# OminiX-ai/OminiX-MLX

Hardware: AMD Instinct MI355X
Metric: decode_tokens_per_sec (higher is better)
Workload: dtype bf16

## Files before the change

include/omx.h:

```cpp
#ifndef OMX_H
#define OMX_H

#include <stddef.h>
#include <stdint.h>

#ifdef __cplusplus
extern "C" {
#endif

typedef enum omx_dtype_ {
    OMX_BOOL = 0, OMX_UINT8 = 1, OMX_UINT16 = 2, OMX_UINT32 = 3, OMX_UINT64 = 4,
    OMX_INT8 = 5, OMX_INT16 = 6, OMX_INT32 = 7, OMX_INT64 = 8,
    OMX_FLOAT16 = 9, OMX_FLOAT32 = 10, OMX_FLOAT64 = 11, OMX_BFLOAT16 = 12, OMX_COMPLEX64 = 13
} omx_dtype;

typedef void* omx_stream;

const char* omx_version(void);
int omx_experiments_built(void);
typedef void (*omx_error_handler_func)(const char* msg, void* data);
void omx_set_error_handler(omx_error_handler_func handler, void* data, void (*dtor)(void*));
const char* omx_last_error(void);
void omx_clear_error(void);
int omx_device_count(int* count);
// ... 200 lines not shown
int omx_debug_attn_step(omx_attn_step_dbg* a, omx_stream stream);
typedef struct omx_gemv_rows_seg_ { const void* w; const void* bias; void* out; int cols, ld; } omx_gemv_rows_seg;
typedef struct omx_gemv_rows_dbg_ {
    const void* x; int M, K, segmented;
    const void* w; const void* bias; const void* resid; const void* gate; int relu, N; void* out;
    omx_gemv_rows_seg seg[3]; int n_plain;
    const void* w_gate; const void* w_up; void* out_act; int half, ld_act, act_mode;
    const void* pre_norm_w; float pre_norm_eps;
    int route_rpw;
} omx_gemv_rows_dbg;
int omx_debug_gemv_rows(omx_gemv_rows_dbg* a, omx_stream stream);
int omx_qwen3_stream(omx_qwen3 m, omx_stream* s);
int omx_qwen3_step_bytes(omx_qwen3 m, int ctx, double* bytes);
int omx_qwen3_decode_path(omx_qwen3 m, int* path);
int omx_qwen3_debug_trace_step(omx_qwen3 m, unsigned long long* host, size_t n_words, int* blocks);
int omx_qwen3_time_step_kernels(omx_qwen3 m, int steps, float* us);
int omx_qwen3_debug_trace_engine(omx_qwen3 m, unsigned long long* host, size_t n_words, int* cus);
int omx_qwen3_debug_step_forms(omx_qwen3 m, int* forms);
int omx_qwen3_debug_raise_give_up(omx_qwen3 m);

int omx_quantize(void* packed, void* scales, void* biases, const void* w, int64_t rows, int cols, int group_size, int bits,
                 omx_dtype dtype, omx_stream stream);
int omx_dequantize(void* out, const void* packed, const void* scales, const void* biases , int64_t rows,
                   int cols, int group_size, int bits, omx_dtype dtype, omx_stream stream);
int omx_quantized_matmul(void* out, const void* x, const void* packed, const void* scales, const void* biases, int M, int N,
                         int K, int group_size, int bits, omx_dtype dtype, omx_stream stream);
int omx_quantized_linear_mfma(void* out, const void* x, const void* packed, const void* scales, const void* biases, const void* resid,
                              const void* gate, int M, int N, int K, int group_size, int bits, omx_stream stream);
int omx_quantized_linear_swiglu(void* out_plain, void* out_act, const void* x, const void* packed, const void* scales, const void* biases,
                                int M, int n_plain, int half, int K, int group_size, int bits, omx_stream stream);
// ... 196 lines not shown
```

ominix-mlx_amd/csrc/attn.hpp:

```cpp
#pragma once
#include "common.hpp"

namespace omx {

struct AttnDecodeArgs {
    const bf16_t* q;
    const bf16_t* k;
    const bf16_t* v;
    int64_t kv_batch_stride, kv_head_stride;
    int B, H, Hkv, Tk;
    float scale;
    int mask_mode;
    const void* mask;
    int nsplit;
    float* ws_o;
    float* ws_ml;
    bf16_t* out;
    int64_t q_bs, q_hs;
    int causal_tail;
};

constexpr int kAttnTraceWords = 16;
struct AttnStepArgs {
    const bf16_t* qkv;
    bf16_t* k;
    bf16_t* v;
    int64_t kv_head_stride;
    int H, Hkv, cap;
    float scale, eps;
    const bf16_t* q_norm_w;
    const bf16_t* k_norm_w;
    const float* rope_cur;
    const int* pos_ptr;
    const unsigned* seq_ptr;
    unsigned tag_mul, tag_add;
    int chunk;
    int nsplit;
// ... 6 lines not shown
    bf16_t* o_out;
    float* o_out_f32;
    int o_rows;
    int o_rpw, o_nhi;
    uint64_t* xg;
    const uint32_t* o_wq;
    const uint32_t* o_sb;
    int o_group;
    int f16;
    const bf16_t* gu_gate;
    const bf16_t* gu_up;
    const bf16_t* gu_norm_w;
    bf16_t* gu_out;
    int gu_rows;
    uint64_t* hg;
    const bf16_t* dn_w;
    bf16_t* dn_out;
    uint64_t* ag;
    uint64_t* rg;
    const bf16_t* nq_w0;
    const bf16_t* nq_w1;
    const bf16_t* nq_w2;
    int nq_n0, nq_n1, nq_rows;
    const bf16_t* nq_norm_w;
    const bf16_t* nq_bias;
    bf16_t* nq_out;
};
bool attn_step_down_ok(int o_rows, int gu_rows, int nq_rows);
bool attn_step_oproj_ok(int H, int Hkv, int D, int nsplit, int o_rows);
bool attn_step_gateup_ok(int H, int Hkv, int D, int nsplit, int o_rows, int gu_rows);
// ... 12 lines not shown
```

ominix-mlx_amd/csrc/attn_step.hip:

```cpp
#include <algorithm>

#include "attn.hpp"
#include "act16.hpp"
#include "gemv_parts.hpp"
#include "granule.hpp"
#include "launch_timing.hpp"

namespace omx {

namespace {

constexpr int kBlock = 512;
constexpr int kWaves = 8;
constexpr unsigned kSpinLimit = 1u << 15;

template <int N>
__device__ __forceinline__ float swap_halves(float v) {
    if (N == 16) return dpp_f<0x128>(v);
    return dpp_f<0x1B>(dpp_f<kDppHalfMirror>(v));
}

template <bool F16 = false>
__device__ __forceinline__ void unpack8(const u32x4 r, float (&x)[8]) {
#pragma unroll
// ... 89 lines not shown
    return d;
}

__device__ __forceinline__ float dot8_chain(const u32x4 w, const u32x4 xp, float acc) {
#pragma unroll
    for (int i = 0; i < 4; ++i) {
        acc = fmaf(bf16lo(w[i]), bf16lo(xp[i]), acc);
        acc = fmaf(bf16hi(w[i]), bf16hi(xp[i]), acc);
    }
    return acc;
}

constexpr int kORows = 4;

constexpr int kGuBlockPairs = 48, kGuHidden = 4096, kGuNV = kGuHidden / 512;
enum { kGuTicket = 0, kGuReduced = 1, kGuWords = 4 };

__device__ __forceinline__ int gateup_claim(int* sm_gu, int lane) {
    int t = 0;
    if (lane == 0) t = __hip_atomic_fetch_add(sm_gu + kGuTicket, 1, __ATOMIC_RELAXED, __HIP_MEMORY_SCOPE_WORKGROUP);
    return __builtin_amdgcn_readfirstlane(t);
}

__device__ __forceinline__ void gateup_issue(const AttnStepArgs& a, u32x4 (*w)[kGuNV], int pair, int lane) {
    const u32x4* g = reinterpret_cast<const u32x4*>(a.gu_gate + (size_t)pair * kGuHidden);
    const u32x4* u = reinterpret_cast<const u32x4*>(a.gu_up + (size_t)pair * kGuHidden);
#pragma unroll
    for (int j = 0; j < kGuNV; ++j) {
        w[0][j] = ld_nt(g + j * 64 + lane);
        w[1][j] = ld_nt(u + j * 64 + lane);
    }
    __builtin_amdgcn_sched_barrier(0);
}

template <int NVW>
__device__ __forceinline__ void oproj_await_vector(const AttnStepArgs& a, u32x4* sm_x, unsigned tag, int lane, int wave) {
    asm volatile("s_waitcnt vmcnt(0)" ::: "memory");
    if (wave == 0) {
        constexpr int SEGS = NVW * 8;
        const uint64_t* probe = a.xg + (size_t)min(lane, SEGS - 1) * 32 + 31;
        for (unsigned spins = 0; spins < kSpinLimit; ++spins) {
            const unsigned long long g = ld_granule(probe);
            if (__all((unsigned)(g >> 32) == tag)) break;
            __builtin_amdgcn_s_sleep(4);
        }
    }
    __syncthreads();
// ... 255 lines not shown
            }
        if (TRACE) __hip_atomic_fetch_add(sm_gu + kDnStored, stored, __ATOMIC_RELAXED, __HIP_MEMORY_SCOPE_WORKGROUP);
    }
    if constexpr (TRACE) {
        lds_barrier();
        if (threadIdx.x == 0) {
            tr[14] = wall_clock64();
            tr[15] = (unsigned long long)sm_gu[kDnReduced] | (unsigned long long)sm_gu[kDnStored] << 32;
        }
    }
}

template <bool TRACE, bool DN = false>
__device__ __forceinline__ void gateup_phase(const AttnStepArgs& a, u32x4* xs, float* red, int* sm_gu, const uint16_t* sm_pub, unsigned tag,
                                             int lane, int wave, int pub_row0, int pub_rows, unsigned long long* tr,
                                             unsigned char* sm_dn = nullptr) {
    typedef Act16<false> A;
    const int pair0 = ((int)blockIdx.y * (int)gridDim.x + (int)blockIdx.x) * kGuBlockPairs;
    uint16_t* park = DN ? reinterpret_cast<uint16_t*>(sm_dn + kDnParkOff) : nullptr;
    constexpr int PV = kGuNV * 64 / 256;
    u32x4 nwv[PV];
#pragma unroll
    for (int i = 0; i < PV; ++i) nwv[i] = *(reinterpret_cast<const u32x4*>(a.gu_norm_w) + (threadIdx.x & 255) + i * 256);
    u32x4 wA[2][kGuNV], wB[2][kGuNV];
    int tA = 0, tB;
    if (wave != 0) {
        tA = gateup_claim(sm_gu, lane);
        gateup_issue(a, wA, pair0 + tA, lane);
    }
    lds_barrier();
    if (wave == 0) {
// ... 41 lines not shown
        gateup_issue(a, wB, pair0 + tB, lane);
    }
    lds_barrier();
    unsigned res2 = 0;
    if constexpr (DN) res2 = reinterpret_cast<const unsigned*>(xs)[(pair0 / kGuBlockPairs) * (kDnBlockRows / 2) + (lane & (kDnBlockRows / 2 - 1))];
    rmsnorm_in_lds<A, PV>(xs, red, nwv, kGuHidden, a.eps, threadIdx.x < 256);
    if (wave == 0) {
        gateup_issue(a, wB, pair0 + tB, lane);
        gateup_reduce<DN>(a, wA, xs, pair0 + tA, lane, park + tA);
        if (TRACE && threadIdx.x == 0) tr[7] = wall_clock64();
        asm volatile("; first pair reduced: wave 0, its second pair just asked for" ::: "memory");
    } else {
        gateup_reduce<DN>(a, wA, xs, pair0 + tA, lane, park + tA);
        asm volatile("; first pair reduced: the second pair came in through the hop" ::: "memory");
    }
    int n_reduced = 1;
    int nA = gateup_claim(sm_gu, lane), nB;
    for (;;) {
        if (nA >= kGuBlockPairs) {
            gateup_reduce<DN>(a, wB, xs, pair0 + tB, lane, park + tB);
            ++n_reduced;
            break;
        }
        tA = nA;
        gateup_issue(a, wA, pair0 + tA, lane);
        nB = gateup_claim(sm_gu, lane);
        gateup_reduce<DN>(a, wB, xs, pair0 + tB, lane, park + tB);
        if (nB >= kGuBlockPairs) {
            gateup_reduce<DN>(a, wA, xs, pair0 + tA, lane, park + tA);
            n_reduced += 2;
            break;
        }
        tB = nB;
        gateup_issue(a, wB, pair0 + tB, lane);
        nA = gateup_claim(sm_gu, lane);
        gateup_reduce<DN>(a, wA, xs, pair0 + tA, lane, park + tA);
        n_reduced += 2;
    }
    if constexpr (TRACE) {
        if (lane == 0) {
            __hip_atomic_fetch_add(sm_gu + kGuReduced, n_reduced, __ATOMIC_RELAXED, __HIP_MEMORY_SCOPE_WORKGROUP);
            if (wave == 0) tr[8] = wall_clock64();
            if (wave == kWaves - 1) tr[9] = wall_clock64();
        }
        lds_barrier();
        if (threadIdx.x == 0) tr[10] = (unsigned long long)sm_gu[kGuReduced];
    }
    if constexpr (DN) down_qkv_phase<TRACE>(a, sm_dn, xs, red, sm_gu, res2, tag, lane, wave, tr);
}

template <int NVW, int R, bool GU = false>
__device__ __forceinline__ void oproj_phase(const AttnStepArgs& a, u32x4* sm_x, unsigned tag, int lane, int wave, int o_row0,
                                            unsigned long long* tr, uint16_t* sm_pub = nullptr, int pub_row0 = 0) {
    u32x4 ow[R][NVW];
#pragma unroll
    for (int r = 0; r < R; ++r) {
        const int row = min(o_row0 + r, a.o_rows - 1);
        const u32x4* p = reinterpret_cast<const u32x4*>(a.o_w + (size_t)row * (NVW * 512));
#pragma unroll
        for (int j = 0; j < NVW; ++j) ow[r][j] = __builtin_nontemporal_load(p + j * 64 + lane);
    }
    bf16_t o_res[R];
#pragma unroll
    for (int r = 0; r < R; ++r) o_res[r] = a.o_resid[min(o_row0 + r, a.o_rows - 1)];
    __builtin_amdgcn_sched_barrier(0);
    oproj_await_vector<NVW>(a, sm_x, tag, lane, wave);
    if (tr && threadIdx.x == 0) tr[5] = wall_clock64();
    float acc[R];
#pragma unroll
    for (int r = 0; r < R; ++r) acc[r] = 0.f;
#pragma unroll
    for (int j = 0; j < NVW; ++j) {
        const u32x4 xp = sm_x[j * 64 + lane];
#pragma unroll
        for (int r = 0; r < R; ++r) acc[r] = dot8_chain(ow[r][j], xp, acc[r]);
    }
#pragma unroll
    for (int r = 0; r < R; ++r) acc[r] = wave_sum(acc[r]);
    if (lane == 0) {
#pragma unroll
// ... 105 lines not shown
    static_assert(!GU || (NVW == kGuNV && D == 128), "gate/up follows the bf16 O projection of hidden 4096 only");
    typedef Act16<F16> A16;
    constexpr int LPR = D / 8;
    constexpr int TPW = 64 / LPR;
    constexpr bool QO = NVW >= 100;
    constexpr int NV = QO ? NVW - 100 : NVW;
    constexpr bool OPROJ = NV > 0;
    extern __shared__ __attribute__((aligned(16))) unsigned char smem[];
    float* sm_o = reinterpret_cast<float*>(smem);
    float* sm_m = sm_o + kWaves * TPW * GT * D;
    float* sm_l = sm_m + kWaves * GT;
    u32x4* sm_q = reinterpret_cast<u32x4*>(sm_l + kWaves * GT);
    u32x4* sm_x = sm_q + (GT + 1) * LPR;
    float* sm_xsum = reinterpret_cast<float*>(sm_x + NV * 64);
    int* sm_gu = reinterpret_cast<int*>(sm_x + NV * 64);

    const int lane = threadIdx.x & 63;
    const int wave = threadIdx.x >> 6;
    const int c = lane % LPR;
    const int sg = lane / LPR;
    const int kvh = blockIdx.x, split = blockIdx.y;
    const int G = a.H / a.Hkv;
    unsigned long long* tr = TRACE ? a.trace + ((size_t)split * a.Hkv + kvh) * kAttnTraceWords : nullptr;
    if (TRACE && threadIdx.x == 0) tr[0] = wall_clock64();
    if constexpr (GU) {
        if (threadIdx.x < (DN ? kDnWords : kGuWords)) sm_gu[threadIdx.x] = 0;
    }

    bf16_t* Kb = a.k + (size_t)kvh * a.kv_head_stride;
    bf16_t* Vb = a.v + (size_t)kvh * a.kv_head_stride;
// ... 122 lines not shown
#pragma unroll
            for (int e = 0; e < 4; ++e) o[g][e] *= al;
#pragma unroll
            for (int u = 0; u < kKU; ++u) {
                const float p = (mn == -INFINITY) ? 0.f : __expf(s[u][g] - mn);
                l[g] += p;
                const f32x2 pp = {p, p};
#pragma unroll
                for (int e = 0; e < 4; ++e) o[g][e] = __builtin_elementwise_fma(pp, vf[u][e], o[g][e]);
            }
        }
    };
    if (wave < n_units && t_begin + wave * TPW < t_end) round(wave);
    for (int u0 = wave + kWaves * kKU; u0 < n_units && t_begin + u0 * TPW < t_end; u0 += kWaves * kKU) round(u0);
    if (TRACE && threadIdx.x == 0) tr[2] = wall_clock64();

    if (active) {
#pragma unroll
        for (int g = 0; g < GT; ++g) {
            float* dst = sm_o + (((size_t)(wave * TPW + sg) * GT + g) * D + c * 8);
            *reinterpret_cast<f32x4*>(dst) = f32x4{o[g][0][0], o[g][0][1], o[g][1][0], o[g][1][1]};
            *reinterpret_cast<f32x4*>(dst + 4) = f32x4{o[g][2][0], o[g][2][1], o[g][3][0], o[g][3][1]};
            float lw = readlane_f(l[g], 0);
#pragma unroll
            for (int r = 1; r < TPW; ++r) lw += readlane_f(l[g], r * LPR);
            if (lane == 0) {
                sm_m[wave * GT + g] = m[g];
                sm_l[wave * GT + g] = lw;
            }
        }
        __syncthreads();
        if (TRACE && !GU && threadIdx.x == 0) tr[7] = wall_clock64();
        for (int idx = threadIdx.x; idx < G * D; idx += kBlock) {
            const int g = idx / D, d = idx % D;
            float M = sm_m[g];
#pragma unroll
            for (int w = 1; w < kWaves; ++w) M = fmaxf(M, sm_m[w * GT + g]);
            float L = 0.f, O = 0.f;
#pragma unroll
            for (int w = 0; w < kWaves; ++w) {
                const float mw = sm_m[w * GT + g];
                const float f = (mw == -INFINITY) ? 0.f : __expf(mw - M);
                float ow = 0.f;
#pragma unroll
                for (int r = 0; r < TPW; ++r) ow += sm_o[((size_t)(w * TPW + r) * GT + g) * D + d];
                L = fmaf(f, sm_l[w * GT + g], L);
// ... 9 lines not shown
    }
    if (TRACE && threadIdx.x == 0) tr[3] = wall_clock64();

    if (OPROJ && split >= G) {
        const int g = ((split - G) * (int)gridDim.x + kvh) * kWaves + wave;
        const bool hi = g < a.o_nhi;
        const int rows = hi ? a.o_rpw : a.o_rpw - 1;
        const int o_row0 = hi ? g * a.o_rpw : a.o_nhi * a.o_rpw + (g - a.o_nhi) * (a.o_rpw - 1);
        unsigned long long* otr = TRACE ? tr : nullptr;
        if constexpr (GU) {
            auto row0_of = [&](int w) { return w < a.o_nhi ? w * a.o_rpw : a.o_nhi * a.o_rpw + (w - a.o_nhi) * (a.o_rpw - 1); };
            const int pub_row0 = row0_of(g - wave), pub_rows = row0_of(g - wave + kWaves) - pub_row0;
            uint16_t* sm_pub = reinterpret_cast<uint16_t*>(sm_l);
            if (rows == 2) oproj_phase<NV, 2, true>(a, sm_x, tag, lane, wave, o_row0, otr, sm_pub, pub_row0);
            else oproj_phase<NV, 3, true>(a, sm_x, tag, lane, wave, o_row0, otr, sm_pub, pub_row0);
            gateup_phase<TRACE, DN>(a, sm_x, sm_m, sm_gu, sm_pub, tag, lane, wave, pub_row0, pub_rows, otr, smem);
            return;
        } else
        if constexpr (QO) {
            if (rows <= 1) oproj_phase_q4<NV, 1>(a, sm_x, sm_xsum, tag, lane, wave, o_row0, otr);
            else if (rows == 2) oproj_phase_q4<NV, 2>(a, sm_x, sm_xsum, tag, lane, wave, o_row0, otr);
            else if (rows == 3) oproj_phase_q4<NV, 3>(a, sm_x, sm_xsum, tag, lane, wave, o_row0, otr);
            else oproj_phase_q4<NV, 4>(a, sm_x, sm_xsum, tag, lane, wave, o_row0, otr);
        } else {
            if (rows <= 1) oproj_phase<(NV > 0 ? NV : 1), 1>(a, sm_x, tag, lane, wave, o_row0, otr);
            else if (rows == 2) oproj_phase<(NV > 0 ? NV : 1), 2>(a, sm_x, tag, lane, wave, o_row0, otr);
            else if (rows == 3) oproj_phase<(NV > 0 ? NV : 1), 3>(a, sm_x, tag, lane, wave, o_row0, otr);
            else oproj_phase<(NV > 0 ? NV : 1), 4>(a, sm_x, tag, lane, wave, o_row0, otr);
        }
        return;
    }

    if (split < G && wave < D / 64) {
        const int head = kvh * G + split;
        const uint64_t* base = a.ws + (size_t)head * a.nsplit * (D + 2);
        bf16_t* out = a.out + (size_t)head * D;
        const int dim = wave * 64 + lane;
        const int nb = (a.nsplit + 15) / 16;
        uint64_t* xg_head = OPROJ ? a.xg + (size_t)head * (D / 2) : nullptr;
        if (nb <= 1) gather_head<D, 1, F16>(a, base, n_active, tag, lane, dim, out, xg_head);
        else if (nb == 2) gather_head<D, 2, F16>(a, base, n_active, tag, lane, dim, out, xg_head);
        else gather_head<D, 3, F16>(a, base, n_active, tag, lane, dim, out, xg_head);
        if (TRACE && threadIdx.x == 0) tr[4] = wall_clock64();
    }
    if constexpr (GU) {
        lds_barrier();
        gateup_phase<TRACE, DN>(a, sm_x, sm_m, sm_gu, nullptr, tag, lane, wave, 0, 0, TRACE ? tr : nullptr, smem);
    }
}

}

int attn_step_block_tokens(int D) { return 64 / (D / 8); }

constexpr int kMaxSplits = 48;
void attn_step_plan(int tk_max, int Hkv, int G, int D, int* chunk, int* nsplit) {
    const int unit = attn_step_block_tokens(D);
    int target = std::max(1, std::min(kMaxSplits, 256 / std::max(Hkv, 1)));
    if (const char* v = getenv("OMX_ATTN_STEP_SPLITS")) target = std::max(1, std::min(kMaxSplits, atoi(v)));
    int ch = unit * ((tk_max + unit * target - 1) / (unit * target));
    if (ch < unit) ch = unit;
    int ns = (tk_max + ch - 1) / ch;
// ... 43 lines not shown
    if (qo)
        OMX_REQUIRE(!a.o_w && a.o_sb && a.o_out && !a.o_out_f32 && attn_step_oproj_q4_ok(a.H, a.Hkv, D, a.nsplit, a.o_rows, a.o_group),
                    "decode attention + packed O projection: shape does not qualify (H*D = %d, group %d)", a.H * D, a.o_group);
    if (a.o_w || qo) {
        OMX_REQUIRE(a.o_resid && (a.o_out || a.o_out_f32) && a.xg && attn_step_oproj_ok(a.H, a.Hkv, D, a.nsplit, a.o_rows),
                    "decode attention + O projection: shape does not qualify (H*D = %d, %d rows, %d blocks)", a.H * D, a.o_rows, a.Hkv * a.nsplit);
        nvw = a.H * D / 512;
        a.o_rpw = oproj_rows_per_wave(a.H, a.Hkv, a.nsplit, a.o_rows);
        const int waves = (a.Hkv * a.nsplit - a.H) * kWaves;
        a.o_nhi = a.o_rpw > 1 ? a.o_rows - waves * (a.o_rpw - 1) : waves;
    }
    if (a.gu_gate)
        OMX_REQUIRE(a.o_w && a.o_out && !a.o_out_f32 && !a.f16 && a.gu_up && a.gu_norm_w && a.gu_out && a.hg &&
                        attn_step_gateup_ok(a.H, a.Hkv, D, a.nsplit, a.o_rows, a.gu_rows),
                    "decode attention + gate/up: shape does not qualify (%d blocks, %d O rows, %d pairs)", a.Hkv * a.nsplit, a.o_rows, a.gu_rows);
    if (a.dn_w)
        OMX_REQUIRE(a.gu_gate && a.dn_out && a.ag && a.rg && a.nq_w0 && a.nq_w1 && a.nq_w2 && a.nq_norm_w && a.nq_out &&
                        a.nq_n0 > 0 && a.nq_n1 > 0 && a.nq_rows > a.nq_n0 + a.nq_n1 && attn_step_down_ok(a.o_rows, a.gu_rows, a.nq_rows),
                    "decode attention + down + q/k/v: shape does not qualify (%d rows, %d pairs, %d q/k/v rows)", a.o_rows, a.gu_rows, a.nq_rows);
    const dim3 grid(a.Hkv, a.nsplit), block(kBlock);
    const int gt = G <= 1 ? 1 : G <= 2 ? 2 : G <= 4 ? 4 : 8;
#define OMX_ATTN_LAUNCH(DD, GG, TT, NN)                                                                                  \
    {                                                                                                                    \
        if (shmem > 48 * 1024)                                                                                           \
            OMX_HIP_CHECK(hipFuncSetAttribute((const void*)attn_step_kernel<DD, GG, TT, NN>,                            \
                                              hipFuncAttributeMaxDynamicSharedMemorySize, (int)shmem));                  \
        OMX_LAUNCH_TIMED((attn_step_kernel<DD, GG, TT, NN>), grid, block, shmem, s, a);                                  \
        OMX_LAUNCH_CHECK();                                                                                              \
        return 0;                                                                                                        \
    }
// ... 5 lines not shown
        OMX_LAUNCH_CHECK();                                                                                              \
        return 0;                                                                                                        \
    }
#define OMX_ATTN_LAUNCH_DN(TT)                                                                                           \
    {                                                                                                                    \
        OMX_HIP_CHECK(hipFuncSetAttribute((const void*)attn_step_kernel<128, 4, TT, kGuNV, false, true, true>,           \
                                          hipFuncAttributeMaxDynamicSharedMemorySize, (int)shmem));                      \
        OMX_LAUNCH_TIMED((attn_step_kernel<128, 4, TT, kGuNV, false, true, true>), grid, block, shmem, s, a);            \
        OMX_LAUNCH_CHECK();                                                                                              \
        return 0;                                                                                                        \
    }
#define OMX_ATTN_STEP_CASE(DD, GG)                                                                                       \
    if (D == DD && gt == GG) {                                                                                           \
        const size_t shmem = ((size_t)kWaves * (64 / (DD / 8)) * GG * DD + 2 * kWaves * GG) * sizeof(float) +            \
                             (size_t)(GG + 1) * (DD / 8) * 16 + (size_t)nvw * 64 * 16 + (qo ? (size_t)nvw * 64 : 0) +    \
                             (a.dn_w ? kDnWords * sizeof(int) : a.gu_gate ? kGuWords * sizeof(int) : 0);                 \
        if (a.gu_gate) {                            \
            if constexpr (DD == 128 && GG == 4) {                                                                        \
                static_assert(kDnLdsBytes <= kWaves * 4 * 4 * 128 * 4, "the down phase lives in the split-merge area");  \
                if (a.dn_w && a.trace) OMX_ATTN_LAUNCH_DN(true)                                                          \
                if (a.dn_w) OMX_ATTN_LAUNCH_DN(false)                                                                    \
                if (a.trace) OMX_ATTN_LAUNCH_GU(true)                                                                    \
                OMX_ATTN_LAUNCH_GU(false)                                                                                \
            }                                                                                                            \
            return set_error("decode attention + gate/up: no instantiation for head_dim %d, group %d", DD, GG);         \
        }                                                                                                                \
        if (a.trace && !qo) {                           \
            if (nvw == 0) OMX_ATTN_LAUNCH(DD, GG, true, 0)                                                               \
            if (nvw == 8) OMX_ATTN_LAUNCH(DD, GG, true, 8)                                                               \
            return set_error("decode attention: no traced instantiation for H*D = %d", a.H * DD);                       \
        }                                                                                                                \
// ... 35 lines not shown
```

ominix-mlx_amd/csrc/engine.hip:

```cpp
#include "engine_model.hpp"

namespace omx {
namespace {

__global__ void rope_table_kernel(float* cos_t, float* sin_t, int cap, int half, double neg_log_base_over_half,
                                  double scale) {
    const int idx = blockIdx.x * blockDim.x + threadIdx.x;
    if (idx >= cap * half) return;
    const int t = idx / half, i = idx % half;
    const double ang = ((double)t * scale) * exp((double)i * neg_log_base_over_half);
    double s, c;
    sincos(ang, &s, &c);
    cos_t[idx] = (float)c;
    sin_t[idx] = (float)s;
}


}
}

extern "C" {

int omx_qwen3_create(omx_qwen3* out, const omx_qwen3_config* cfg) {
    OMX_REQUIRE(out && cfg, "omx_qwen3_create: null argument");
// ... 602 lines not shown
    return 0;
}

int omx_qwen3_last_decode_ms(omx_qwen3 m, float* ms) {
    OMX_REQUIRE(m && ms, "omx_qwen3_last_decode_ms: null argument");
    *ms = m->last_decode_ms;
    return 0;
}

int omx_qwen3_stream(omx_qwen3 m, omx_stream* s) {
    OMX_REQUIRE(m && s, "omx_qwen3_stream: null argument");
    *s = (omx_stream)m->stream;
    return 0;
}

int omx_qwen3_debug_trace_step(omx_qwen3 m, unsigned long long* host, size_t n_words, int* blocks) {
    OMX_REQUIRE(m && host && blocks, "omx_qwen3_debug_trace_step: null argument");
    StepState st;
    if (read_step_state(m, &st)) return 1;
    if (prepare_step(m, st.pos)) return 1;
    const size_t per_layer = (size_t)m->attn_nsplit * m->Hkv * kAttnTraceWords, need = per_layer * m->cfg.num_hidden_layers;
    OMX_REQUIRE(n_words >= need, "omx_qwen3_debug_trace_step: buffer of %zu words, need %zu", n_words, need);
    unsigned long long* dev = nullptr;
    OMX_HIP_CHECK(hipMalloc(&dev, need * 8));
    OMX_HIP_CHECK(hipMemsetAsync(dev, 0, need * 8, m->stream));
    m->attn_trace = dev;
    const int rc = enqueue_step(m, true);
    m->attn_trace = nullptr;
    if (!rc) {
        OMX_HIP_CHECK(hipStreamSynchronize(m->stream));
        OMX_HIP_CHECK(hipMemcpy(host, dev, need * 8, hipMemcpyDeviceToHost));
    }
    (void)hipFree(dev);
    *blocks = m->attn_nsplit * m->Hkv;
    return rc ? 1 : step_health(m);
}

int omx_qwen3_time_step_kernels(omx_qwen3 m, int steps, float* us) {
    OMX_REQUIRE(m && us && steps > 0, "omx_qwen3_time_step_kernels: bad arguments");
    OMX_REQUIRE(!m->cfg.quant_bits && m->cfg.num_experts == 0 && m->allreduce == nullptr, "omx_qwen3_time_step_kernels: dense bf16 single-rank models only");
    const int L = m->cfg.num_hidden_layers;
    std::vector<hipEvent_t> ev((size_t)(L * kLayerClasses + 2) * 2);
    for (auto& e : ev) OMX_HIP_CHECK(hipEventCreate(&e));
    double sum[KC_COUNT] = {};
    int rc = 0;
    bool fused_o = false, engine = false, hybrid = false, chain = false;
    const double o_bytes = (double)m->H * m->cfg.head_dim * m->cfg.hidden_size, gu_bytes = 2.0 * m->cfg.hidden_size * m->I;
    const double qkv_bytes = (double)(m->H + 2 * m->Hkv) * m->cfg.head_dim * m->cfg.hidden_size, down_bytes = (double)m->cfg.hidden_size * m->I;
    arm_launch_events(nullptr, nullptr);
    for (int it = 0; it < steps && !rc; ++it) {
// ... 109 lines not shown
```

ominix-mlx_amd/csrc/engine_model.hpp:

```cpp
#pragma once
#include <math.h>
#include <stdlib.h>
#include <string.h>

#include <algorithm>
#include <map>
#include <string>
#include <vector>

#include "attn.hpp"
#include "workspace.hpp"
#include "step_state.hpp"
#include "gemm.hpp"
#include "gemv.hpp"
#include "random.hpp"
#include "sample_filter.hpp"
#include "logprob.hpp"
#include "prefill.hpp"
#include "quant.hpp"
#include "launch_timing.hpp"
#include "aql_step.hpp"
#include "act16.hpp"
#include "peer.hpp"
#include "step_engine.hpp"
// ... 203 lines not shown
std::pair<int, int> quant_format_of(omx_qwen3 m, const std::string& prefix);

void drop_graphs(omx_qwen3 m);
void recapture_step(omx_qwen3 m);
int rank_allreduce(omx_qwen3 m, void* buf, size_t n, int dtype, int op);
int allreduce_sum(omx_qwen3 m, float* buf, size_t n);
int read_step_state(omx_qwen3 m, StepState* st);
int write_step_state(omx_qwen3 m, const StepState& st);
int reset_sampler_history(omx_qwen3 m);
bool sampling_penalised(const omx_sampling& p);
bool attention_takes_oproj(omx_qwen3 m, int layer);
bool any_layer_takes_oproj(omx_qwen3 m);
bool down_takes_qkv(omx_qwen3 m);
bool attention_takes_gateup(omx_qwen3 m, int layer);
bool attention_takes_down(omx_qwen3 m, int layer);
int step_engine_mode(omx_qwen3 m);
bool step_engine_takes(omx_qwen3 m);
int step_aql_mode(omx_qwen3 m);
int enqueue_step(omx_qwen3 m, bool with_head);
int enqueue_step_tail(omx_qwen3 m, bool with_head, const bf16_t* h, const float* pending, int pending_n, bool tp);
int context_bucket(omx_qwen3 m, int tk);
int prepare_step(omx_qwen3 m, int pos);
int run_step(omx_qwen3 m, bool with_head, int pos);
int step_gave_up(omx_qwen3 m, unsigned* code);
int step_health(omx_qwen3 m);
int step_fallback(omx_qwen3 m, const StepState& st);
int launch_ep_fold(int grid, bf16_t* out, const bf16_t* resid, const float* partial, int64_t n, bool f16, hipStream_t s);

int prefill_reserve(omx_qwen3 m, int T, bool dequant = true);
void dq_cache_prepare(omx_qwen3 m);
// ... 15 lines not shown
```

ominix-mlx_amd/csrc/engine_step.hip:

```cpp
#include "engine_model.hpp"

namespace omx {
namespace {

__device__ __forceinline__ void step_begin(const StepState* st, unsigned* seq, float* rope_cur, const float* rope_cos,
                                           const float* rope_sin, int half) {
    if (blockIdx.x != 0) return;
    if (seq && threadIdx.x == 0) *seq += 1u;
    if (rope_cur && (int)threadIdx.x < 2 * half) {
        const int t = threadIdx.x, pos = st->pos;
        rope_cur[t] = t < half ? rope_cos[(size_t)pos * half + t] : rope_sin[(size_t)pos * half + t - half];
    }
}

template <int BITS>
__global__ __launch_bounds__(256) void qembed_kernel(bf16_t* __restrict__ h, const uint32_t* __restrict__ w,
                                                     const bf16_t* __restrict__ scales, const bf16_t* __restrict__ biases,
                                                     const StepState* st, int hidden, int group, unsigned* seq, float* rope_cur,
                                                     const float* rope_cos, const float* rope_sin, int half, bool scales_f16) {
    constexpr int EPW = 32 / BITS;
    step_begin(st, seq, rope_cur, rope_cos, rope_sin, half);
    const size_t row = st->cur_token;
    const int words = hidden / EPW;
    for (int i = blockIdx.x * blockDim.x + threadIdx.x; i < words; i += gridDim.x * blockDim.x) {
// ... 206 lines not shown

bool attention_takes_gateup(omx_qwen3 m, int layer) {
    const bool off = env_off("OMX_ATTN_GATEUP");
    const omx_qwen3_config& c = m->cfg;
    if (off || m->gateup_disabled || c.quant_bits != 0 || m->f16 || c.num_experts > 0 || c.tp_size > 1 || c.ep_size > 1 || m->allreduce != nullptr) return false;
    if (step_engine_mode(m) != 0 || env_int("OMX_GEMV_RPW_O", 0) != 0 || env_int("OMX_GEMV_RPW_GU", 0) != 0) return false;
    if (!m->gateup_gran || m->cus < 256 || !attention_takes_oproj(m, layer)) return false;
    return attn_step_gateup_ok(m->H, m->Hkv, c.head_dim, m->attn_nsplit, c.hidden_size, m->I);
}

bool attention_takes_down(omx_qwen3 m, int layer) {
    const bool off = env_off("OMX_ATTN_DOWN");
    const omx_qwen3_config& c = m->cfg;
    if (off || !m->act_gran || layer + 1 >= c.num_hidden_layers || !attention_takes_gateup(m, layer) || !down_takes_qkv(m)) return false;
    return attn_step_down_ok(c.hidden_size, m->I, (m->H + 2 * m->Hkv) * c.head_dim);
}

static bool peer_fused_fits(omx_qwen3 m, int N, int K) {
    return m->peer_dev != nullptr && gemv_grid(N, K, EPI_F32, 0) <= 2 * m->cus;
}

static int enqueue_attention(omx_qwen3 m, int l, hipStream_t s, const bf16_t* resid = nullptr, bf16_t* out = nullptr, float* out_f32 = nullptr,
                             bool gateup = false, bool down = false) {
    const omx_qwen3_config& c = m->cfg;
    const int D = c.head_dim;
    const LayerW& L = m->layers[l];
    AttnStepArgs a = {};
    a.qkv = m->qkv;
    a.k = m->kcache[l]; a.v = m->vcache[l];
    a.kv_head_stride = (int64_t)m->cap * D;
// ... 11 lines not shown
    a.abort_flag = m->wait_abort;
    a.trace = m->attn_trace ? m->attn_trace + (size_t)l * m->attn_nsplit * m->Hkv * kAttnTraceWords : nullptr;
    a.f16 = m->f16;
    if (resid && (out || out_f32)) {
        a.o_resid = resid; a.o_out = out; a.o_out_f32 = out_f32; a.o_rows = c.hidden_size; a.xg = m->attn_xg;
        if (c.quant_bits) {
            const QMat& o = m->qlayers[l].o;
            a.o_wq = o.w; a.o_sb = o.sb; a.o_group = o.group;
        } else {
            a.o_w = L.o;
        }
    }
    if (gateup) {
        a.gu_gate = L.gate; a.gu_up = L.up; a.gu_norm_w = L.post_ln; a.gu_out = m->act; a.gu_rows = m->I;
        a.hg = m->gateup_gran;
    }
    if (down) {
        const LayerW& Ln = m->layers[l + 1];
        a.dn_w = L.down; a.dn_out = const_cast<bf16_t*>(resid);
        a.ag = m->act_gran; a.rg = m->chain_gran;
        a.nq_w0 = Ln.q; a.nq_w1 = Ln.k; a.nq_w2 = Ln.v;
        a.nq_n0 = m->H * D; a.nq_n1 = m->Hkv * D; a.nq_rows = (m->H + 2 * m->Hkv) * D;
        a.nq_norm_w = Ln.in_ln; a.nq_bias = Ln.qkv_bias; a.nq_out = m->qkv;
    }
    return launch_attn_step(a, D, s);
}

int enqueue_step_tail(omx_qwen3 m, bool with_head, const bf16_t* h, const float* pending, int pending_n, bool tp) {
    const omx_qwen3_config& c = m->cfg;
    hipStream_t s = m->stream;
// ... 491 lines not shown
```

ominix-mlx_amd/engine.py:

```python
from __future__ import annotations

import ctypes
import sys
from typing import Dict, Iterator, Optional

import numpy as np

from . import OmxError, Sampling, check, lib, require_device
from .ops import Tensor

c_int, c_float, c_void_p, c_uint32 = ctypes.c_int, ctypes.c_float, ctypes.c_void_p, ctypes.c_uint32


class Qwen3Config(ctypes.Structure):
    _fields_ = [("hidden_size", c_int), ("num_hidden_layers", c_int), ("intermediate_size", c_int),
                ("num_attention_heads", c_int), ("num_key_value_heads", c_int), ("head_dim", c_int),
                ("vocab_size", c_int), ("rms_norm_eps", c_float), ("rope_theta", c_float), ("rope_scale", c_float),
                ("tie_word_embeddings", c_int), ("max_context", c_int), ("tp_rank", c_int), ("tp_size", c_int),
                ("quant_bits", c_int), ("quant_group", c_int), ("num_experts", c_int), ("num_experts_per_tok", c_int),
                ("moe_intermediate_size", c_int), ("moe_mode", c_int), ("norm_topk_prob", c_int), ("no_qk_norm", c_int),
                ("ep_rank", c_int), ("ep_size", c_int), ("attention_bias", c_int), ("quant_scales_f16", c_int),
                ("float16_weights", c_int)]


# ... 70 lines not shown
    "omx_qwen3_prefill_embeds": (c_int, [c_void_p, ctypes.POINTER(c_uint32), c_int, c_void_p, c_int, c_int, c_int, ctypes.POINTER(c_uint32)]),
    "omx_qwen3_decode": (c_int, [c_void_p, c_int, ctypes.POINTER(c_uint32)]),
    "omx_qwen3_last_logits": (c_int, [c_void_p, c_void_p, c_int]),
    "omx_qwen3_set_logprobs": (c_int, [c_void_p, c_int]),
    "omx_qwen3_decode_logprobs": (c_int, [c_void_p, c_int, ctypes.POINTER(c_uint32), ctypes.POINTER(c_float), c_void_p, c_void_p]),
    "omx_qwen3_last_logprobs": (c_int, [c_void_p, ctypes.POINTER(c_float), c_void_p, c_void_p]),
    "omx_qwen3_last_decode_ms": (c_int, [c_void_p, ctypes.POINTER(c_float)]),
    "omx_qwen3_last_prefill_ms": (c_int, [c_void_p, ctypes.POINTER(c_float)]),
    "omx_qwen3_dequant_bytes": (c_int, [c_void_p, ctypes.POINTER(ctypes.c_size_t)]),
    "omx_qwen3_debug_read": (c_int, [c_void_p, ctypes.c_char_p, c_void_p, ctypes.c_size_t]),
    "omx_qwen3_debug_write": (c_int, [c_void_p, ctypes.c_char_p, c_void_p, ctypes.c_size_t]),
    "omx_qwen3_stream": (c_int, [c_void_p, ctypes.POINTER(c_void_p)]),
    "omx_qwen3_step_bytes": (c_int, [c_void_p, c_int, ctypes.POINTER(ctypes.c_double)]),
    "omx_qwen3_decode_path": (c_int, [c_void_p, ctypes.POINTER(c_int)]),
    "omx_qwen3_debug_trace_step": (c_int, [c_void_p, c_void_p, ctypes.c_size_t, ctypes.POINTER(c_int)]),
    "omx_qwen3_time_step_kernels": (c_int, [c_void_p, c_int, ctypes.POINTER(ctypes.c_float)]),
    "omx_qwen3_debug_trace_engine": (c_int, [c_void_p, c_void_p, ctypes.c_size_t, ctypes.POINTER(c_int)]),
    "omx_qwen3_debug_step_forms": (c_int, [c_void_p, ctypes.POINTER(c_int)]),
    "omx_qwen3_debug_raise_give_up": (c_int, [c_void_p]),
    "omx_qwen3_verify": (c_int, [c_void_p, ctypes.POINTER(c_uint32), c_int, ctypes.POINTER(c_uint32)]),
    "omx_qwen3_verify_logits": (c_int, [c_void_p, c_int, c_void_p, c_int]),
    "omx_qwen3_trim": (c_int, [c_void_p, c_int, c_uint32]),
    "omx_qwen3_score": (c_int, [c_void_p, ctypes.POINTER(c_uint32), c_int, ctypes.POINTER(c_uint32), ctypes.POINTER(c_float), ctypes.POINTER(c_uint32)]),
    "omx_qwen3_last_score_ms": (c_int, [c_void_p, ctypes.POINTER(c_float), ctypes.POINTER(c_float)]),
    "omx_qwen3_get_weight": (c_int, [c_void_p, ctypes.c_char_p, ctypes.POINTER(c_void_p), ctypes.POINTER(ctypes.c_size_t)]),
    "omx_qwen3_set_quant_format": (c_int, [c_void_p, ctypes.c_char_p, c_int, c_int]),
    "omx_qwen3_quant_format": (c_int, [c_void_p, ctypes.c_char_p, ctypes.POINTER(c_int), ctypes.POINTER(c_int)]),
    "omx_qwen3_batch_create": (c_int, [ctypes.POINTER(c_void_p), c_void_p, c_int, c_int]),
    "omx_qwen3_batch_destroy": (c_int, [c_void_p]),
    "omx_qwen3_batch_set_sampler": (c_int, [c_void_p, c_int, ctypes.c_float, ctypes.c_uint64]),
# ... 433 lines not shown
    def decode_path(self) -> str:
        v = c_int()
        check(lib.omx_qwen3_decode_path(self._h, ctypes.byref(v)))
        path = ("unbuilt", "graph", "eager", "aql")[v.value & 0xFF]
        return path + "".join(" " + name for bit, name in enumerate(("gateup_disabled", "chain_disabled", "engine_disabled", "oproj_disabled"))
                              if v.value >> (8 + bit) & 1)

    KERNEL_CLASSES = ("qkv", "attention", "o", "gate_up", "down", "lm_head", "step_engine")

    def time_step_kernels(self, steps: int = 4) -> dict:
        us = (ctypes.c_float * 7)()
        check(lib.omx_qwen3_time_step_kernels(self._h, steps, us))
        return dict(zip(self.KERNEL_CLASSES, (float(v) for v in us)))

    def step_forms(self) -> dict:
        f = (c_int * 7)()
        check(lib.omx_qwen3_debug_step_forms(self._h, f))
        return {"down_qkv": bool(f[0]), "attn_oproj": bool(f[1]), "step_engine": int(f[2]), "down_qkv_gave_up": bool(f[3]),
                "attn_gateup": bool(f[4]), "attn_gateup_gave_up": bool(f[5]), "attn_down": bool(f[6])}

    def raise_give_up(self) -> None:
        check(lib.omx_qwen3_debug_raise_give_up(self._h))

    def step_bytes(self, ctx: int) -> float:
        v = ctypes.c_double()
        check(lib.omx_qwen3_step_bytes(self._h, ctx, ctypes.byref(v)))
        return v.value

    def batch(self, n_slots: int, max_context: int = 0, kv_bits: int = 0) -> "Batch":
        return Batch(self, n_slots, max_context, kv_bits)


class Batch:

# ... 167 lines not shown
```

Before: 352.6.

## Prefetch tail gate/up weight pairs into LDS during attention phase

```diff
diff --git a/include/omx.h b/include/omx.h
--- a/include/omx.h
+++ b/include/omx.h
@@ -238,6 +238,7 @@
 int omx_qwen3_step_bytes(omx_qwen3 m, int ctx, double* bytes);
 int omx_qwen3_decode_path(omx_qwen3 m, int* path);
 int omx_qwen3_debug_trace_step(omx_qwen3 m, unsigned long long* host, size_t n_words, int* blocks);
+int omx_qwen3_debug_trace_step_wide(omx_qwen3 m, unsigned long long* host, size_t n_words, int* blocks, int* words);
 int omx_qwen3_time_step_kernels(omx_qwen3 m, int steps, float* us);
 int omx_qwen3_debug_trace_engine(omx_qwen3 m, unsigned long long* host, size_t n_words, int* cus);
 int omx_qwen3_debug_step_forms(omx_qwen3 m, int* forms);
diff --git a/ominix-mlx_amd/csrc/attn.hpp b/ominix-mlx_amd/csrc/attn.hpp
--- a/ominix-mlx_amd/csrc/attn.hpp
+++ b/ominix-mlx_amd/csrc/attn.hpp
@@ -20,7 +20,9 @@
     int causal_tail;
 };
 
-constexpr int kAttnTraceWords = 16;
+constexpr int kAttnTraceWords = 18;
+constexpr int kAttnTraceHostWords = 16;
+constexpr int kGuParkMax = 5;
 struct AttnStepArgs {
     const bf16_t* qkv;
     bf16_t* k;
@@ -57,6 +59,7 @@
     bf16_t* gu_out;
     int gu_rows;
     uint64_t* hg;
+    int gu_parked;
     const bf16_t* dn_w;
     bf16_t* dn_out;
     uint64_t* ag;
diff --git a/ominix-mlx_amd/csrc/attn_step.hip b/ominix-mlx_amd/csrc/attn_step.hip
--- a/ominix-mlx_amd/csrc/attn_step.hip
+++ b/ominix-mlx_amd/csrc/attn_step.hip
@@ -127,7 +127,7 @@
 constexpr int kORows = 4;
 
 constexpr int kGuBlockPairs = 48, kGuHidden = 4096, kGuNV = kGuHidden / 512;
-enum { kGuTicket = 0, kGuReduced = 1, kGuWords = 4 };
+enum { kGuTicket = 0, kGuReduced = 1, kGuUnparked = 2, kGuWords = 4 };
 
 __device__ __forceinline__ int gateup_claim(int* sm_gu, int lane) {
     int t = 0;
@@ -144,6 +144,30 @@
         w[1][j] = ld_nt(u + j * 64 + lane);
     }
     __builtin_amdgcn_sched_barrier(0);
+}
+
+constexpr int kGuPairBytes = 2 * kGuHidden * 2;
+__device__ __forceinline__ void gateup_park_issue(const AttnStepArgs& a, unsigned char* sm_park, int pair0, int lane, int wave) {
+    __builtin_amdgcn_s_waitcnt(0x0F70);
+    const int first = pair0 + kGuBlockPairs - a.gu_parked;
+    const unsigned dst0 = (unsigned)(uintptr_t)sm_park + (unsigned)__builtin_amdgcn_readfirstlane(wave) * 1024u;
+    const unsigned off = (unsigned)(wave * 64 + lane) * 16u;
+    for (int i = 0; i < 2 * a.gu_parked; ++i) {
+        const bf16_t* row = ((i & 1) ? a.gu_up : a.gu_gate) + (size_t)(first + (i >> 1)) * kGuHidden;
+        const unsigned dst = dst0 + (unsigned)i * (kGuHidden * 2);
+        unsigned keep;
+        asm volatile("s_nop 4\n\ts_mov_b32 %0, m0\n\ts_mov_b32 m0, %3\n\ts_nop 0\n\tglobal_load_lds_dwordx4 %1, %2 nt\n\ts_mov_b32 m0, %0"
+                     : "=&s"(keep) : "v"(off), "s"(row), "s"(dst) : "memory");
+    }
+}
+
+__device__ __forceinline__ void gateup_unpark(const unsigned char* sm_park, u32x4 (*w)[kGuNV], int slot, int lane) {
+    const u32x4* p = reinterpret_cast<const u32x4*>(sm_park + (size_t)slot * kGuPairBytes);
+#pragma unroll
+    for (int r = 0; r < 2; ++r) {
+#pragma unroll
+        for (int j = 0; j < kGuNV; ++j) w[r][j] = p[(r * kGuNV + j) * 64 + lane];
+    }
 }
 
 template <int NVW>
@@ -429,7 +453,7 @@
 template <bool TRACE, bool DN = false>
 __device__ __forceinline__ void gateup_phase(const AttnStepArgs& a, u32x4* xs, float* red, int* sm_gu, const uint16_t* sm_pub, unsigned tag,
                                              int lane, int wave, int pub_row0, int pub_rows, unsigned long long* tr,
-                                             unsigned char* sm_dn = nullptr) {
+                                             unsigned char* sm_dn, const unsigned char* sm_rows) {
     typedef Act16<false> A;
     const int pair0 = ((int)blockIdx.y * (int)gridDim.x + (int)blockIdx.x) * kGuBlockPairs;
     uint16_t* park = DN ? reinterpret_cast<uint16_t*>(sm_dn + kDnParkOff) : nullptr;
@@ -501,21 +525,24 @@
         gateup_reduce<DN>(a, wA, xs, pair0 + tA, lane, park + tA);
         asm volatile("; first pair reduced: the second pair came in through the hop" ::: "memory");
     }
-    int n_reduced = 1;
-    int nA = gateup_claim(sm_gu, lane), nB;
+    const int hbm = kGuBlockPairs - a.gu_parked;
+    int n_reduced = 1, n_unparked = 0;
+    int nA = gateup_claim(sm_gu, lane), nB, nP;
     for (;;) {
-        if (nA >= kGuBlockPairs) {
+        if (nA >= hbm) {
             gateup_reduce<DN>(a, wB, xs, pair0 + tB, lane, park + tB);
             ++n_reduced;
+            nP = nA;
             break;
         }
         tA = nA;
         gateup_issue(a, wA, pair0 + tA, lane);
         nB = gateup_claim(sm_gu, lane);
         gateup_reduce<DN>(a, wB, xs, pair0 + tB, lane, park + tB);
-        if (nB >= kGuBlockPairs) {
+        if (nB >= hbm) {
             gateup_reduce<DN>(a, wA, xs, pair0 + tA, lane, park + tA);
             n_reduced += 2;
+            nP = nB;
             break;
         }
         tB = nB;
@@ -524,14 +551,23 @@
         gateup_reduce<DN>(a, wA, xs, pair0 + tA, lane, park + tA);
         n_reduced += 2;
     }
+    for (; nP < kGuBlockPairs; nP = gateup_claim(sm_gu, lane)) {
+        gateup_unpark(sm_rows, wA, nP - hbm, lane);
+        gateup_reduce<DN>(a, wA, xs, pair0 + nP, lane, park + nP);
+        ++n_unparked;
+    }
     if constexpr (TRACE) {
         if (lane == 0) {
-            __hip_atomic_fetch_add(sm_gu + kGuReduced, n_reduced, __ATOMIC_RELAXED, __HIP_MEMORY_SCOPE_WORKGROUP);
+            __hip_atomic_fetch_add(sm_gu + kGuReduced, n_reduced + n_unparked, __ATOMIC_RELAXED, __HIP_MEMORY_SCOPE_WORKGROUP);
+            __hip_atomic_fetch_add(sm_gu + kGuUnparked, n_unparked, __ATOMIC_RELAXED, __HIP_MEMORY_SCOPE_WORKGROUP);
             if (wave == 0) tr[8] = wall_clock64();
             if (wave == kWaves - 1) tr[9] = wall_clock64();
         }
         lds_barrier();
-        if (threadIdx.x == 0) tr[10] = (unsigned long long)sm_gu[kGuReduced];
+        if (threadIdx.x == 0) {
+            tr[10] = (unsigned long long)sm_gu[kGuReduced];
+            tr[17] = (unsigned long long)sm_gu[kGuUnparked];
+        }
     }
     if constexpr (DN) down_qkv_phase<TRACE>(a, sm_dn, xs, red, sm_gu, res2, tag, lane, wave, tr);
 }
@@ -551,6 +587,10 @@
 #pragma unroll
     for (int r = 0; r < R; ++r) o_res[r] = a.o_resid[min(o_row0 + r, a.o_rows - 1)];
     __builtin_amdgcn_sched_barrier(0);
+    if constexpr (GU) if (tr) {
+        asm volatile("s_waitcnt vmcnt(%0)" ::"n"(R * NVW + R) : "memory");
+        if (threadIdx.x == 0) tr[16] = wall_clock64();
+    }
     oproj_await_vector<NVW>(a, sm_x, tag, lane, wave);
     if (tr && threadIdx.x == 0) tr[5] = wall_clock64();
     float acc[R];
@@ -686,6 +726,7 @@
     u32x4* sm_x = sm_q + (GT + 1) * LPR;
     float* sm_xsum = reinterpret_cast<float*>(sm_x + NV * 64);
     int* sm_gu = reinterpret_cast<int*>(sm_x + NV * 64);
+    unsigned char* sm_rows = reinterpret_cast<unsigned char*>(sm_gu + (DN ? kDnWords : kGuWords));
 
     const int lane = threadIdx.x & 63;
     const int wave = threadIdx.x >> 6;
@@ -838,6 +879,7 @@
     if (wave < n_units && t_begin + wave * TPW < t_end) round(wave);
     for (int u0 = wave + kWaves * kKU; u0 < n_units && t_begin + u0 * TPW < t_end; u0 += kWaves * kKU) round(u0);
     if (TRACE && threadIdx.x == 0) tr[2] = wall_clock64();
+    if constexpr (GU) gateup_park_issue(a, sm_rows, (split * (int)gridDim.x + kvh) * kGuBlockPairs, lane, wave);
 
     if (active) {
 #pragma unroll
@@ -853,7 +895,8 @@
                 sm_l[wave * GT + g] = lw;
             }
         }
-        __syncthreads();
+        if constexpr (GU) lds_barrier();
+        else __syncthreads();
         if (TRACE && !GU && threadIdx.x == 0) tr[7] = wall_clock64();
         for (int idx = threadIdx.x; idx < G * D; idx += kBlock) {
             const int g = idx / D, d = idx % D;
@@ -893,7 +936,7 @@
             uint16_t* sm_pub = reinterpret_cast<uint16_t*>(sm_l);
             if (rows == 2) oproj_phase<NV, 2, true>(a, sm_x, tag, lane, wave, o_row0, otr, sm_pub, pub_row0);
             else oproj_phase<NV, 3, true>(a, sm_x, tag, lane, wave, o_row0, otr, sm_pub, pub_row0);
-            gateup_phase<TRACE, DN>(a, sm_x, sm_m, sm_gu, sm_pub, tag, lane, wave, pub_row0, pub_rows, otr, smem);
+            gateup_phase<TRACE, DN>(a, sm_x, sm_m, sm_gu, sm_pub, tag, lane, wave, pub_row0, pub_rows, otr, smem, sm_rows);
             return;
         } else
         if constexpr (QO) {
@@ -923,8 +966,10 @@
         if (TRACE && threadIdx.x == 0) tr[4] = wall_clock64();
     }
     if constexpr (GU) {
+        asm volatile("s_waitcnt vmcnt(0)" ::: "memory");
+        if (TRACE && threadIdx.x == 0) tr[16] = wall_clock64();
         lds_barrier();
-        gateup_phase<TRACE, DN>(a, sm_x, sm_m, sm_gu, nullptr, tag, lane, wave, 0, 0, TRACE ? tr : nullptr, smem);
+        gateup_phase<TRACE, DN>(a, sm_x, sm_m, sm_gu, nullptr, tag, lane, wave, 0, 0, TRACE ? tr : nullptr, smem, sm_rows);
     }
 }
 
@@ -998,6 +1043,8 @@
         OMX_REQUIRE(a.o_w && a.o_out && !a.o_out_f32 && !a.f16 && a.gu_up && a.gu_norm_w && a.gu_out && a.hg &&
                         attn_step_gateup_ok(a.H, a.Hkv, D, a.nsplit, a.o_rows, a.gu_rows),
                     "decode attention + gate/up: shape does not qualify (%d blocks, %d O rows, %d pairs)", a.Hkv * a.nsplit, a.o_rows, a.gu_rows);
+    OMX_REQUIRE(a.gu_parked >= 0 && a.gu_parked <= (a.gu_gate ? kGuParkMax : 0), "decode attention + gate/up: %d parked pairs (0 .. %d, with gate/up in the launch only)",
+                a.gu_parked, kGuParkMax);
     if (a.dn_w)
         OMX_REQUIRE(a.gu_gate && a.dn_out && a.ag && a.rg && a.nq_w0 && a.nq_w1 && a.nq_w2 && a.nq_norm_w && a.nq_out &&
                         a.nq_n0 > 0 && a.nq_n1 > 0 && a.nq_rows > a.nq_n0 + a.nq_n1 && attn_step_down_ok(a.o_rows, a.gu_rows, a.nq_rows),
@@ -1033,7 +1080,8 @@
     if (D == DD && gt == GG) {                                                                                           \
         const size_t shmem = ((size_t)kWaves * (64 / (DD / 8)) * GG * DD + 2 * kWaves * GG) * sizeof(float) +            \
                              (size_t)(GG + 1) * (DD / 8) * 16 + (size_t)nvw * 64 * 16 + (qo ? (size_t)nvw * 64 : 0) +    \
-                             (a.dn_w ? kDnWords * sizeof(int) : a.gu_gate ? kGuWords * sizeof(int) : 0);                 \
+                             (a.dn_w ? kDnWords * sizeof(int) : a.gu_gate ? kGuWords * sizeof(int) : 0) +                \
+                             (a.gu_gate ? (size_t)a.gu_parked * kGuPairBytes : 0);                                       \
         if (a.gu_gate) {                            \
             if constexpr (DD == 128 && GG == 4) {                                                                        \
                 static_assert(kDnLdsBytes <= kWaves * 4 * 4 * 128 * 4, "the down phase lives in the split-merge area");  \
diff --git a/ominix-mlx_amd/csrc/engine.hip b/ominix-mlx_amd/csrc/engine.hip
--- a/ominix-mlx_amd/csrc/engine.hip
+++ b/ominix-mlx_amd/csrc/engine.hip
@@ -640,13 +640,13 @@
     return 0;
 }
 
-int omx_qwen3_debug_trace_step(omx_qwen3 m, unsigned long long* host, size_t n_words, int* blocks) {
-    OMX_REQUIRE(m && host && blocks, "omx_qwen3_debug_trace_step: null argument");
+static int trace_step(omx_qwen3 m, unsigned long long* host, size_t n_words, int* blocks, int host_words, const char* who) {
+    OMX_REQUIRE(m && host && blocks, "%s: null argument", who);
     StepState st;
     if (read_step_state(m, &st)) return 1;
     if (prepare_step(m, st.pos)) return 1;
-    const size_t per_layer = (size_t)m->attn_nsplit * m->Hkv * kAttnTraceWords, need = per_layer * m->cfg.num_hidden_layers;
-    OMX_REQUIRE(n_words >= need, "omx_qwen3_debug_trace_step: buffer of %zu words, need %zu", n_words, need);
+    const size_t records = (size_t)m->attn_nsplit * m->Hkv * m->cfg.num_hidden_layers, need = records * kAttnTraceWords;
+    OMX_REQUIRE(n_words >= records * host_words, "%s: buffer of %zu words, need %zu", who, n_words, records * host_words);
     unsigned long long* dev = nullptr;
     OMX_HIP_CHECK(hipMalloc(&dev, need * 8));
     OMX_HIP_CHECK(hipMemsetAsync(dev, 0, need * 8, m->stream));
@@ -655,11 +655,21 @@
     m->attn_trace = nullptr;
     if (!rc) {
         OMX_HIP_CHECK(hipStreamSynchronize(m->stream));
-        OMX_HIP_CHECK(hipMemcpy(host, dev, need * 8, hipMemcpyDeviceToHost));
+        OMX_HIP_CHECK(hipMemcpy2D(host, (size_t)host_words * 8, dev, (size_t)kAttnTraceWords * 8, (size_t)host_words * 8, records, hipMemcpyDeviceToHost));
     }
     (void)hipFree(dev);
     *blocks = m->attn_nsplit * m->Hkv;
     return rc ? 1 : step_health(m);
+}
+
+int omx_qwen3_debug_trace_step(omx_qwen3 m, unsigned long long* host, size_t n_words, int* blocks) {
+    return trace_step(m, host, n_words, blocks, kAttnTraceHostWords, "omx_qwen3_debug_trace_step");
+}
+
+int omx_qwen3_debug_trace_step_wide(omx_qwen3 m, unsigned long long* host, size_t n_words, int* blocks, int* words) {
+    OMX_REQUIRE(words, "omx_qwen3_debug_trace_step_wide: null argument");
+    *words = kAttnTraceWords;
+    return trace_step(m, host, n_words, blocks, kAttnTraceWords, "omx_qwen3_debug_trace_step_wide");
 }
 
 int omx_qwen3_time_step_kernels(omx_qwen3 m, int steps, float* us) {
diff --git a/ominix-mlx_amd/csrc/engine_model.hpp b/ominix-mlx_amd/csrc/engine_model.hpp
--- a/ominix-mlx_amd/csrc/engine_model.hpp
+++ b/ominix-mlx_amd/csrc/engine_model.hpp
@@ -241,6 +241,7 @@
 bool down_takes_qkv(omx_qwen3 m);
 bool attention_takes_gateup(omx_qwen3 m, int layer);
 bool attention_takes_down(omx_qwen3 m, int layer);
+int gateup_parked_pairs(omx_qwen3 m, int layer);
 int step_engine_mode(omx_qwen3 m);
 bool step_engine_takes(omx_qwen3 m);
 int step_aql_mode(omx_qwen3 m);
diff --git a/ominix-mlx_amd/csrc/engine_step.hip b/ominix-mlx_amd/csrc/engine_step.hip
--- a/ominix-mlx_amd/csrc/engine_step.hip
+++ b/ominix-mlx_amd/csrc/engine_step.hip
@@ -244,6 +244,12 @@
     const omx_qwen3_config& c = m->cfg;
     if (off || !m->act_gran || layer + 1 >= c.num_hidden_layers || !attention_takes_gateup(m, layer) || !down_takes_qkv(m)) return false;
     return attn_step_down_ok(c.hidden_size, m->I, (m->H + 2 * m->Hkv) * c.head_dim);
+}
+
+constexpr int kGuParkDefault = 3;
+int gateup_parked_pairs(omx_qwen3 m, int layer) {
+    const int n = env_int("OMX_ATTN_PARK", kGuParkDefault);
+    return attention_takes_gateup(m, layer) ? std::max(0, std::min(kGuParkMax, n)) : 0;
 }
 
 static bool peer_fused_fits(omx_qwen3 m, int N, int K) {
@@ -285,6 +291,7 @@
     if (gateup) {
         a.gu_gate = L.gate; a.gu_up = L.up; a.gu_norm_w = L.post_ln; a.gu_out = m->act; a.gu_rows = m->I;
         a.hg = m->gateup_gran;
+        a.gu_parked = gateup_parked_pairs(m, l);
     }
     if (down) {
         const LayerW& Ln = m->layers[l + 1];
diff --git a/ominix-mlx_amd/engine.py b/ominix-mlx_amd/engine.py
--- a/ominix-mlx_amd/engine.py
+++ b/ominix-mlx_amd/engine.py
@@ -108,6 +108,7 @@
     "omx_qwen3_step_bytes": (c_int, [c_void_p, c_int, ctypes.POINTER(ctypes.c_double)]),
     "omx_qwen3_decode_path": (c_int, [c_void_p, ctypes.POINTER(c_int)]),
     "omx_qwen3_debug_trace_step": (c_int, [c_void_p, c_void_p, ctypes.c_size_t, ctypes.POINTER(c_int)]),
+    "omx_qwen3_debug_trace_step_wide": (c_int, [c_void_p, c_void_p, ctypes.c_size_t, ctypes.POINTER(c_int), ctypes.POINTER(c_int)]),
     "omx_qwen3_time_step_kernels": (c_int, [c_void_p, c_int, ctypes.POINTER(ctypes.c_float)]),
     "omx_qwen3_debug_trace_engine": (c_int, [c_void_p, c_void_p, ctypes.c_size_t, ctypes.POINTER(c_int)]),
     "omx_qwen3_debug_step_forms": (c_int, [c_void_p, ctypes.POINTER(c_int)]),
@@ -571,10 +572,10 @@
         return dict(zip(self.KERNEL_CLASSES, (float(v) for v in us)))
 
     def step_forms(self) -> dict:
-        f = (c_int * 7)()
+        f = (c_int * 8)()
         check(lib.omx_qwen3_debug_step_forms(self._h, f))
         return {"down_qkv": bool(f[0]), "attn_oproj": bool(f[1]), "step_engine": int(f[2]), "down_qkv_gave_up": bool(f[3]),
-                "attn_gateup": bool(f[4]), "attn_gateup_gave_up": bool(f[5]), "attn_down": bool(f[6])}
+                "attn_gateup": bool(f[4]), "attn_gateup_gave_up": bool(f[5]), "attn_down": bool(f[6]), "gateup_parked": int(f[7])}
 
     def raise_give_up(self) -> None:
         check(lib.omx_qwen3_debug_raise_give_up(self._h))
```

After: 354.3, median of 6. Within noise of the previous version (+0.5%).
